# nagadomi/nunif

Measured on NVIDIA H100. Metric: waifu2x_input_megapixels_per_sec, higher is better.
Workload: dtype f16

## Files before the change

nunif_b200/csrc/gemm.cu:

```cuda
#include "gemm.h"
#include "gemm_wgmma.cuh"
#include "tmap.h"
#include "../../include/nunif_b200.h"
#include <mutex>
#include <cstdlib>

namespace nb200 {

typedef CUresult (*EncodeTiledFn)(CUtensorMap*, CUtensorMapDataType, cuuint32_t, void*, const cuuint64_t*,
                                  const cuuint64_t*, const cuuint32_t*, const cuuint32_t*, CUtensorMapInterleave,
                                  CUtensorMapSwizzle, CUtensorMapL2promotion, CUtensorMapFloatOOBfill);

static EncodeTiledFn get_encode() {
    static EncodeTiledFn fn = nullptr;
    static std::once_flag once;
    std::call_once(once, [] {
        void* p = nullptr;
        cudaDriverEntryPointQueryResult q;
        if (cudaGetDriverEntryPoint("cuTensorMapEncodeTiled", &p, cudaEnableDefault, &q) == cudaSuccess &&
            q == cudaDriverEntryPointSuccess)
            fn = (EncodeTiledFn)p;
    });
    return fn;
}

int encode(CUtensorMap* m, const void* base, int rank, const cuuint64_t* dims, const cuuint64_t* strides_bytes,
                  const cuuint32_t* box, int swizzle_bytes) {
    EncodeTiledFn fn = get_encode();
    if (!fn) return fail("cuTensorMapEncodeTiled is not available (no CUDA driver?)");
    cuuint32_t estr[5] = {1, 1, 1, 1, 1};
    CUtensorMapSwizzle sw = swizzle_bytes == 128 ? CU_TENSOR_MAP_SWIZZLE_128B
                                                 : (swizzle_bytes == 64 ? CU_TENSOR_MAP_SWIZZLE_64B : CU_TENSOR_MAP_SWIZZLE_32B);
    CUresult r = fn(m, CU_TENSOR_MAP_DATA_TYPE_FLOAT16, (cuuint32_t)rank, const_cast<void*>(base), dims, strides_bytes, box,
                    estr, CU_TENSOR_MAP_INTERLEAVE_NONE, sw, CU_TENSOR_MAP_L2_PROMOTION_L2_256B,
                    CU_TENSOR_MAP_FLOAT_OOB_FILL_NONE);
    if (r != CUDA_SUCCESS) return fail("cuTensorMapEncodeTiled failed with CUresult " + std::to_string((int)r));
    return 0;
}

template <int BN, int BK, bool A2 = false>
static int launch_t(cudaStream_t st, const GemmMaps& maps, const GemmParams& p, int m_tiles, int n_tiles) {
    using Cfg = GemmCfg<BN, BK>;
    if (ensure_dyn_smem((const void*)gemm_conv_kernel<BN, BK, A2>, Cfg::SMEM_BYTES)) return 1;
    cudaLaunchConfig_t cfg = {};
    cfg.gridDim = dim3((unsigned)m_tiles * n_tiles); cfg.blockDim = dim3(GEMM_THREADS); cfg.dynamicSmemBytes = Cfg::SMEM_BYTES;
    cfg.stream = st;
    cudaLaunchAttribute at[1];
    at[0].id = cudaLaunchAttributeProgrammaticStreamSerialization;
    at[0].val.programmaticStreamSerializationAllowed = 1;
    cfg.attrs = at; cfg.numAttrs = 1;
    NB_CUDA(cudaLaunchKernelEx(&cfg, gemm_conv_kernel<BN, BK, A2>, maps, p));
    NB_LAUNCHED();
    return 0;
}

template <int BK>
static int launch_bn(int bn, cudaStream_t st, const GemmMaps& maps, const GemmParams& p, int m_tiles, int n_tiles) {
    if (p.k2) switch (bn) {
        case 64: return launch_t<64, BK, true>(st, maps, p, m_tiles, n_tiles);
        case 96: return launch_t<96, BK, true>(st, maps, p, m_tiles, n_tiles);
        default: return fail("second A operand: unsupported BLOCK_N");
    }
    switch (bn) {
        case 16: return launch_t<16, BK>(st, maps, p, m_tiles, n_tiles);
        case 32: return launch_t<32, BK>(st, maps, p, m_tiles, n_tiles);
        case 48: return launch_t<48, BK>(st, maps, p, m_tiles, n_tiles);
        case 64: return launch_t<64, BK>(st, maps, p, m_tiles, n_tiles);
        case 96: return launch_t<96, BK>(st, maps, p, m_tiles, n_tiles);
        case 128: return launch_t<128, BK>(st, maps, p, m_tiles, n_tiles);
    }
    return fail("unsupported BLOCK_N");
}

static int num_sms() { return device_sm_count(); }

std::atomic<int> g_tune_epoch{0};
int g_tune[16] = {0, 0, 0,  0, 0, 0,  0,
                   0, 0,  0, 0, 0, 0, 0, 0, 0};

static int encode_nhwc4(CUtensorMap* m, const __half* base, int C, int X, int Y, int B, long long sx, long long sy, long long sb,
                        int cw, int tw, int th) {
    cuuint64_t dims[4] = {(cuuint64_t)C, (cuuint64_t)X, (cuuint64_t)Y, (cuuint64_t)B};
    cuuint64_t strides[3] = {(cuuint64_t)sx * 2, (cuuint64_t)sy * 2, (cuuint64_t)sb * 2};
    cuuint32_t box[4] = {(cuuint32_t)cw, (cuuint32_t)tw, (cuuint32_t)th, 1};
    return encode(m, base, 4, dims, strides, box, cw * 2);
}

int conv_gemm(cudaStream_t st, const ConvGemm& g) {
    NB_CHECK(g.A && g.Wt && g.out, "null pointer");
    NB_CHECK(g.Ci % 8 == 0, "input channel stride must be a multiple of 8");
    NB_CHECK(g.N % 16 == 0, "N must be a multiple of 16 (pad the weights)");
    GemmParams p;
    memset(&p, 0, sizeof(p));
    int ktap;
    cuuint64_t dims[5], strides[4];
    cuuint32_t box[5];
    const cuuint64_t e = 2;
    const cuuint64_t rs = (g.a_row_stride ? (cuuint64_t)g.a_row_stride : (cuuint64_t)g.Wi * g.Ci) * e;
    const cuuint64_t is = (g.a_img_stride ? (cuuint64_t)g.a_img_stride * e : (cuuint64_t)g.Hi * rs);
    switch (g.kind) {
        case CG_LINEAR_FLAT: {
            const long long M = (long long)g.B * g.Hi * g.Wi;
            p.B = 1; p.Ho = 1; p.Wo = (int)M; p.TH = 1; p.TW = 128;
            p.taps = g.a_planes; ktap = g.Cin;
            NB_CHECK(g.a_planes >= 1 && g.a_planes <= 16, "bad plane count");
            for (int t = 0; t < p.taps; ++t) { p.tap_dy[t] = 0; p.tap_dx[t] = 0; p.tap_dyi[t] = (int8_t)t; }
            dims[0] = g.Cin; dims[1] = M; dims[2] = g.a_planes; dims[3] = 1; dims[4] = 1;
            strides[0] = g.Ci * e; strides[1] = (g.a_planes > 1 ? (cuuint64_t)g.a_plane_stride : (cuuint64_t)M * g.Ci) * e;
            strides[2] = (cuuint64_t)M * g.Ci * e * g.a_planes; strides[3] = strides[2];
            break;
        }
        case CG_LINEAR_2D:
        case CG_CONV3: {
            const int kk = g.kind == CG_CONV3 ? 3 : 1;
            const int pad = g.kind == CG_CONV3 ? g.pad : 0;
            NB_CHECK(pad == 0 || pad == 1, "conv3x3 padding must be 0 or 1");
            p.B = g.B; p.Ho = g.Hi - (kk - 1) + 2 * pad; p.Wo = g.Wi - (kk - 1) + 2 * pad; p.TH = 8; p.TW = 16;
            p.taps = kk * kk; ktap = g.Cin;
            for (int t = 0; t < p.taps; ++t) { p.tap_dy[t] = (int8_t)(t / kk - pad); p.tap_dx[t] = (int8_t)(t % kk - pad); p.tap_dyi[t] = 0; }
            dims[0] = g.Cin; dims[1] = g.Wi; dims[2] = 1; dims[3] = g.Hi; dims[4] = g.B;
            strides[0] = g.Ci * e; strides[1] = rs; strides[2] = rs;
            strides[3] = is;
            break;
        }
        case CG_TCONV3: {
            NB_CHECK(g.dil >= 1 && g.dil <= 127, "temporal dilation must be in [1, 127]");
            p.B = g.B; p.Ho = g.Hi; p.Wo = g.Wi; p.TH = 8; p.TW = 16;
            p.taps = 3; ktap = g.Cin;
            for (int t = 0; t < 3; ++t) { p.tap_dy[t] = (int8_t)((t - 1) * g.dil); p.tap_dx[t] = 0; p.tap_dyi[t] = 0; }
            dims[0] = g.Cin; dims[1] = g.Wi; dims[2] = 1; dims[3] = g.Hi; dims[4] = g.B;
            strides[0] = g.Ci * e; strides[1] = rs; strides[2] = rs;
            strides[3] = is;
            break;
        }
        case CG_DOWN2: {
            NB_CHECK(g.Hi % 2 == 0 && g.Wi % 2 == 0, "2x2 stride-2 conv needs even H and W");
            NB_CHECK(g.Cin == g.Ci, "2x2 stride-2 conv needs a dense channel dimension");
            p.B = g.B; p.Ho = g.Hi / 2; p.Wo = g.Wi / 2; p.TH = 8; p.TW = 16;
            p.taps = 2; ktap = 2 * g.Cin;
            for (int t = 0; t < 2; ++t) { p.tap_dy[t] = 0; p.tap_dx[t] = 0; p.tap_dyi[t] = t; }
            dims[0] = 2 * g.Cin; dims[1] = g.Wi / 2; dims[2] = 2; dims[3] = g.Hi / 2; dims[4] = g.B;
            strides[0] = 2 * g.Ci * e; strides[1] = rs; strides[2] = 2 * rs;
            strides[3] = is;
            break;
        }
        default: return fail("conv_gemm: unknown kind");
    }
    NB_CHECK(ktap % 32 == 0, "K per tap must be a multiple of 32");
    const bool a2 = g.A2 != nullptr;
    if (a2) {
        NB_CHECK(g.out_mode == OUT_PIXSHUF2 && !g.res, "a second A operand needs the pixel-shuffle output and no residual");
        NB_CHECK(g.Cin2 > 0 && g.Cin2 % 32 == 0 && g.Cin2 <= g.ld2 && g.ld2 % 8 == 0, "second A operand: bad channel count");
    }
    const int BK = (ktap % 64 == 0 && g.Cin2 % 64 == 0) ? 64 : 32;
    p.cpt = ktap / BK;
    p.k2 = a2 ? g.Cin2 / BK : 0;
    p.tiles_x = cdiv(p.Wo, p.TW);
    p.tiles_y = cdiv(p.Ho, p.TH);
    p.N = g.N;
    p.bias = g.bias; p.act = g.act; p.out_mode = g.out_mode; p.cout = g.cout;
    p.has_res = g.res ? 1 : 0;
    p.res_before_act = g.res_before_act;
    const bool shuf = g.out_mode == OUT_PIXSHUF2;
    const bool split = g.out_mode == OUT_SPLIT;
    if (split) {
        NB_CHECK(g.cout % 16 == 0 && g.N % g.cout == 0 && g.N / g.cout <= 4, "split output: N must be 1..4 blocks of cout");
        NB_CHECK(!g.res, "split output does not take a residual");
    }
    if (shuf) {
        NB_CHECK(g.kind != CG_LINEAR_FLAT, "pixel-shuffle output needs 2-D tiling");
        NB_CHECK(g.cout % 16 == 0 && g.N == 4 * g.cout, "pixel-shuffle: N must be 4*cout, cout % 16 == 0");
    }
    NB_CHECK(g.ldo % 8 == 0 && (!g.res || g.ldr % 8 == 0), "channel strides must be multiples of 8");
    int bn = 0, cw = 0;
    static const int cands[] = {128, 96, 64, 48, 32, 16};
    for (int c : cands) {
        const int w = (c % 64 == 0) ? 64 : ((c % 32 == 0) ? 32 : 16);
        if (g.N % c == 0 && (!shuf || g.cout % w == 0) && (!split || g.cout % c == 0) && (!a2 || ((c == 96 || c == 64) && g.cout % c == 0))) {
            bn = c; cw = w; break;
        }
    }
    NB_CHECK(bn > 0, "no BLOCK_N divides N");
    if (!shuf) {
        const long long m_tiles_est = (long long)p.tiles_x * p.tiles_y * p.B;
        static const int narrower[] = {96, 64};
        for (int c : narrower) {
            if ((long long)(g.N / bn) * m_tiles_est >= (long long)num_sms() * 3 / 4) break;
            if (c >= bn || g.N % c) continue;
            const int w = (c % 64 == 0) ? 64 : 32;
            if (split && g.cout % w) continue;
            bn = c; cw = w;
        }
    }
    p.n_tiles = g.N / bn;
    box[0] = BK; box[1] = p.TW; box[2] = 1; box[3] = p.TH; box[4] = 1;
    GemmMaps maps;
    memset(&maps, 0, sizeof(maps));
    if (encode(&maps.a, g.A, 5, dims, strides, box, BK * 2)) return 1;
    const int K = p.taps * ktap + (a2 ? g.Cin2 : 0);
    cuuint64_t bdims[2] = {(cuuint64_t)K, (cuuint64_t)g.N};
    cuuint64_t bstr[1] = {(cuuint64_t)K * e};
    cuuint32_t bbox[2] = {(cuuint32_t)BK, (cuuint32_t)bn};
    if (encode(&maps.b, g.Wt, 2, bdims, bstr, bbox, BK * 2)) return 1;
    if (split) {
        for (int q = 0; q < g.N / g.cout; ++q)
            if (encode_nhwc4(&maps.o[q], g.out + (size_t)q * g.split_stride, g.cout, p.Wo, p.Ho, p.B, g.ldo, (long long)p.Wo * g.ldo,
                             (long long)p.Ho * p.Wo * g.ldo, cw, p.TW, p.TH)) return 1;
    } else if (!shuf) {
        if (encode_nhwc4(&maps.o[0], g.out, g.N, p.Wo, p.Ho, p.B, g.ldo, (long long)p.Wo * g.ldo, (long long)p.Ho * p.Wo * g.ldo,
                         cw, p.TW, p.TH)) return 1;
        if (g.res) {
            const int rW = g.kind == CG_LINEAR_FLAT ? p.Wo : g.res_W, rH = g.kind == CG_LINEAR_FLAT ? 1 : g.res_H;
            p.res_cx = g.kind == CG_LINEAR_FLAT ? 0 : g.res_cx;
            p.res_cy = g.kind == CG_LINEAR_FLAT ? 0 : g.res_cy;
            if (encode_nhwc4(&maps.r[0], g.res, g.N, rW, rH, p.B, g.ldr, (long long)rW * g.ldr, (long long)rH * rW * g.ldr, cw,
                             p.TW, p.TH)) return 1;
        }
    } else {
        const int OW = 2 * p.Wo, OH = 2 * p.Ho;
        for (int q = 0; q < 4; ++q) {
            const int dy = q >> 1, dx = q & 1;
            if (encode_nhwc4(&maps.o[q], g.out + ((size_t)dy * OW + dx) * g.ldo, g.cout, p.Wo, p.Ho, p.B, 2LL * g.ldo,
                             2LL * OW * g.ldo, (long long)OH * OW * g.ldo, cw, p.TW, p.TH)) return 1;
            if (g.res) {
                const int oy = dy + g.res_cy, ox = dx + g.res_cx;
                NB_CHECK(oy + 2 * (p.Ho - 1) < g.res_H && ox + 2 * (p.Wo - 1) < g.res_W, "residual tensor too small");
                if (encode_nhwc4(&maps.r[q], g.res + ((size_t)oy * g.res_W + ox) * g.ldr, g.cout, p.Wo, p.Ho, p.B, 2LL * g.ldr,
                                 2LL * g.res_W * g.ldr, (long long)g.res_H * g.res_W * g.ldr, cw, p.TW, p.TH)) return 1;
            }
        }
        p.res_cx = p.res_cy = 0;
        if (a2) {
            const cuuint64_t px = (cuuint64_t)g.ld2 * e;
            cuuint64_t d2[5] = {(cuuint64_t)g.Cin2, 2, (cuuint64_t)p.Wo, 2, (cuuint64_t)p.B * p.Ho};
            cuuint64_t s2[4] = {px, 2 * px, (cuuint64_t)OW * px, 2 * (cuuint64_t)OW * px};
            cuuint32_t b2[5] = {(cuuint32_t)BK, 1, (cuuint32_t)p.TW, 1, (cuuint32_t)p.TH};
            if (encode(&maps.a2, g.A2, 5, d2, s2, b2, BK * 2)) return 1;
        }
    }
    const int m_tiles = p.tiles_x * p.tiles_y * p.B;
    const double Mrows = (double)p.B * p.Ho * p.Wo;
    const double in_px = g.kind == CG_DOWN2 ? 4.0 * Mrows : ((g.kind == CG_CONV3 || g.kind == CG_TCONV3) ? (double)p.B * g.Hi * g.Wi : Mrows);
    ProfScope ps(st, PC_GEMM, 2.0 * Mrows * (double)g.N * (double)K,
                 in_px * (g.kind == CG_LINEAR_FLAT ? g.Cin * g.a_planes : g.Cin) * 2.0 + (g.res ? Mrows * g.N * 2.0 : 0.0) +
                     4.0 * Mrows * g.Cin2 * (a2 ? 2.0 : 0.0) + (double)g.N * K * 2.0,
                 Mrows * (double)g.N * 2.0);
    if (rec_on()) {
        char line[512];
        snprintf(line, sizeof(line),
                 "gemm,%d,%d,%d,%d,%d,%d,%d,%d,%lld,%lld,%d,%lld,%d,%d,%d,%d,%d,%lld,%d,%d,%d,%d,%d,%d,%d,%d,%d,%d,%d,%d,%d,%d,%d,%d",
                 g.kind, g.pad, g.dil, g.B, g.Hi, g.Wi, g.Ci, g.Cin, g.a_row_stride, g.a_img_stride, g.a_planes, g.a_plane_stride,
                 g.N, g.act, g.ldo, g.out_mode, g.cout, g.split_stride, g.bias ? 1 : 0, g.res ? 1 : 0, g.ldr, g.res_H, g.res_W,
                 g.res_cy, g.res_cx, g.res_before_act, a2 ? 1 : 0, g.Cin2, g.ld2, g.res && (const void*)g.out == (const void*)g.res,
                 (const void*)g.out == (const void*)g.A, bn, BK, m_tiles * p.n_tiles);
        rec_append(line);
    }
    return BK == 64 ? launch_bn<64>(bn, st, maps, p, m_tiles, p.n_tiles) : launch_bn<32>(bn, st, maps, p, m_tiles, p.n_tiles);
}

}

using namespace nb200;

extern "C" int nb200_conv_gemm_f16(const void* A, int B, int Hi, int Wi, int Ci, int Cin, int kind, const void* Wt, int N,
                                   const float* bias, int act, void* out, int ldo, int out_mode, int cout,
                                   const void* res, int ldr, int res_H, int res_W, int res_cy, int res_cx,
                                   int res_before_act, void* stream) {
    ConvGemm g;
    g.A = (const __half*)A; g.B = B; g.Hi = Hi; g.Wi = Wi; g.Ci = Ci; g.Cin = Cin;
    g.kind = kind == 4 ? CG_CONV3 : kind;
    g.pad = kind == 4 ? 1 : 0;
    g.Wt = (const __half*)Wt; g.N = N; g.bias = bias; g.act = act; g.out = (__half*)out; g.ldo = ldo;
    g.out_mode = out_mode; g.cout = cout; g.res = (const __half*)res; g.ldr = ldr; g.res_H = res_H; g.res_W = res_W;
    g.res_cy = res_cy; g.res_cx = res_cx; g.res_before_act = res_before_act;
    return conv_gemm((cudaStream_t)stream, g);
}

extern "C" int nb200_conv_gemm_pixshuf_a2_f16(const void* A, int B, int Hi, int Wi, int Ci, const void* Wt, int N, const float* bias,
                                              int act, void* out, int ldo, int cout, const void* A2, int Cin2, int ld2, void* stream) {
    ConvGemm g;
    g.A = (const __half*)A; g.B = B; g.Hi = Hi; g.Wi = Wi; g.Ci = Ci; g.Cin = Ci; g.kind = CG_LINEAR_2D;
    g.Wt = (const __half*)Wt; g.N = N; g.bias = bias; g.act = act; g.out = (__half*)out; g.ldo = ldo;
    g.out_mode = OUT_PIXSHUF2; g.cout = cout; g.A2 = (const __half*)A2; g.Cin2 = Cin2; g.ld2 = ld2;
    NB_CHECK(g.A2, "null pointer");
    return conv_gemm((cudaStream_t)stream, g);
}

extern "C" int nb200_conv_gemm_ex_f16(const nb200_gemm_desc* d, const void* A, const void* Wt, const float* bias, void* out,
                                      const void* res, const void* A2, void* stream) {
    NB_CHECK(d, "null descriptor");
    ConvGemm g;
    g.A = (const __half*)A; g.B = d->B; g.Hi = d->Hi; g.Wi = d->Wi; g.Ci = d->Ci; g.Cin = d->Cin;
    g.a_row_stride = d->a_row_stride; g.a_img_stride = d->a_img_stride; g.kind = d->kind; g.pad = d->pad; g.dil = d->dil;
    g.Wt = (const __half*)Wt; g.N = d->N; g.bias = bias; g.act = d->act; g.out = (__half*)out; g.ldo = d->ldo;
    g.out_mode = d->out_mode; g.cout = d->cout; g.split_stride = d->split_stride; g.a_planes = d->a_planes;
    g.a_plane_stride = d->a_plane_stride; g.res = (const __half*)res; g.ldr = d->ldr; g.res_H = d->res_H; g.res_W = d->res_W;
    g.res_cy = d->res_cy; g.res_cx = d->res_cx; g.res_before_act = d->res_before_act;
    g.A2 = (const __half*)A2; g.Cin2 = d->Cin2; g.ld2 = d->ld2;
    return conv_gemm((cudaStream_t)stream, g);
}

extern "C" int nb200_tune_set(int key, int value) {
    NB_CHECK(key >= 0 && key < 16, "bad key");
    g_tune[key] = value;
    g_tune_epoch.fetch_add(1);
    return 0;
}
```

nunif_b200/csrc/swin_block.cu:

```cuda
#include "gemm_wgmma.cuh"
#include "swin_kernels.h"
#include "tmap.h"

namespace nb200 {

constexpr int FM_ROWS = 128, FM_STAGES = 5, FM_THREADS = GEMM_CONSUMER_THREADS + 128;
constexpr int FM_PRODUCER_REGS = 40, FM_CONSUMER_REGS = 232;

template <int C>
struct FmCfg {
    static constexpr int KB = C / 32;
    static constexpr int TILE = FM_ROWS * C * 2;
    static constexpr int STAGE = 128 * C;
    static constexpr int SMEM = 2 * TILE + FM_STAGES * STAGE + (2 * FM_STAGES + KB + 1) * 8 + 1024;
};

struct FmMaps {
    CUtensorMap x, att, wp, w1, w2, y, wy;
};

template <int K>
__device__ __forceinline__ float (&half96(float (&acc)[K], int h))[48] { return *reinterpret_cast<float(*)[48]>(&acc[48 * h]); }

__device__ __forceinline__ void wgmma_wait_n(int n) {
    if (n == 0) wgmma_wait<0>();
    else wgmma_wait<1>();
}

template <int C, bool PROJ, int CS>
__global__ void __launch_bounds__(FM_THREADS, 1) swin_mlp_fused_kernel(const __grid_constant__ FmMaps maps, const float* __restrict__ bp,
                                                                     const float* __restrict__ b1, const float* __restrict__ b2,
                                                                     const float* __restrict__ by) {
    using Cfg = FmCfg<C>;
    static_assert(CS % 16 == 0 && 2 * C * CS <= Cfg::STAGE && CS * 256 <= Cfg::TILE, "Wy must fit a ring stage, y the att tile");
    constexpr int KB = Cfg::KB, NP = (KB + 1) / 2, NH = 2 * C / 64, NHALF = C / 96;
    extern __shared__ uint8_t smem_dyn[];
    uint8_t* smem = reinterpret_cast<uint8_t*>((reinterpret_cast<uintptr_t>(smem_dyn) + 1023) & ~(uintptr_t)1023);
    uint8_t* sx = smem;
    uint8_t* satt = smem + Cfg::TILE;
    uint8_t* ring = smem + 2 * Cfg::TILE;
    uint64_t* full = reinterpret_cast<uint64_t*>(ring + FM_STAGES * Cfg::STAGE);
    uint64_t* empty = full + FM_STAGES;
    uint64_t* abar = empty + FM_STAGES;
    uint64_t* xbar = abar + KB;
    const int tid = threadIdx.x, warp = tid >> 5;
    const int row_base = blockIdx.x * FM_ROWS;
    if (tid == GEMM_CONSUMER_THREADS) {
        tma_prefetch_desc(&maps.x);
        tma_prefetch_desc(&maps.w1);
        tma_prefetch_desc(&maps.w2);
        if (CS) tma_prefetch_desc(&maps.wy);
        if (PROJ) {
            tma_prefetch_desc(&maps.att);
            tma_prefetch_desc(&maps.wp);
        }
        for (int s = 0; s < FM_STAGES; ++s) {
            mbar_init(&full[s], 1);
            mbar_init(&empty[s], 2);
        }
        for (int kb = 0; kb < KB; ++kb) mbar_init(&abar[kb], 1);
        mbar_init(xbar, 1);
        fence_barrier_init();
    }
    __syncthreads();

    if (warp >= GEMM_CONSUMER_THREADS / 32) {
        asm volatile("setmaxnreg.dec.sync.aligned.u32 %0;" ::"n"(FM_PRODUCER_REGS));
        if (warp == GEMM_CONSUMER_THREADS / 32 && elect_one()) {
            bool acts = false;
            auto load_acts = [&]() {
                asm volatile("griddepcontrol.wait;" ::: "memory");
                if (PROJ)
                    for (int kb = 0; kb < KB; ++kb) {
                        mbar_expect_tx(&abar[kb], FM_ROWS * 64);
                        tma_load_2d(&maps.att, &abar[kb], satt + kb * (FM_ROWS * 64), kb * 32, row_base);
                    }
                mbar_expect_tx(xbar, Cfg::TILE);
                for (int kb = 0; kb < KB; ++kb) tma_load_2d(&maps.x, xbar, sx + kb * (FM_ROWS * 64), kb * 32, row_base);
                acts = true;
            };
            int it = 0;
            auto push = [&](const CUtensorMap* m, int k0, int n0, int rows, int nbox) {
                if (it == FM_STAGES) load_acts();
                const int s = it % FM_STAGES;
                mbar_wait(&empty[s], ((it / FM_STAGES) & 1) ^ 1);
                mbar_expect_tx(&full[s], nbox * rows * 64);
                for (int b = 0; b < nbox; ++b) tma_load_2d(m, &full[s], ring + s * Cfg::STAGE + b * rows * 64, k0 + 32 * b, n0);
                ++it;
            };
            if (PROJ)
                for (int j = 0; j < NP; ++j) push(&maps.wp, 64 * j, 0, C, min(2, KB - 2 * j));
            push(&maps.w1, 0, 0, 64, KB);
            for (int hc = 0; hc < NH; ++hc) {
                if (hc + 1 < NH) push(&maps.w1, 0, (hc + 1) * 64, 64, KB);
                push(&maps.w2, hc * 64, 0, C, 2);
            }
            if (CS) push(&maps.wy, 0, 0, CS, KB);
            if (!acts) load_acts();
        }
        return;
    }

    asm volatile("setmaxnreg.inc.sync.aligned.u32 %0;" ::"n"(FM_CONSUMER_REGS));
    const int wg = tid >> 7, t = tid & 127;
    const int row0 = wg * 64 + (t >> 5) * 16 + ((t & 31) >> 2);
    const int cq = 2 * (t & 3);
    const uint32_t x_base = smem_u32(sx) + wg * 64 * 64, att_base = smem_u32(satt) + wg * 64 * 64;
    int it = 0, pending = 0;
    auto take = [&]() -> uint32_t {
        const int s = it % FM_STAGES;
        mbar_wait(&full[s], (it / FM_STAGES) & 1);
        return smem_u32(ring + s * Cfg::STAGE);
    };
    auto commit = [&]() {
        wgmma_commit();
        ++it;
        ++pending;
    };
    auto retire = [&](int n) {
        wgmma_wait_n(n);
#pragma unroll
        for (int k = 0; k < FM_STAGES; ++k)
            if (k < pending - n && t == 0) mbar_arrive(&empty[(it - pending + k) % FM_STAGES]);
        pending = min(pending, n);
    };

    if (PROJ) {
        float acc[C / 2];
#pragma unroll
        for (int j = 0; j < C / 2; ++j) acc[j] = 0.f;
        wgmma_fence_operands(acc);
#pragma unroll
        for (int j = 0; j < NP; ++j) {
            const uint32_t bb = take();
#pragma unroll
            for (int kb = 2 * j; kb < 2 * j + 2 && kb < KB; ++kb) mbar_wait(&abar[kb], 0);
            wgmma_fence();
#pragma unroll
            for (int kb = 2 * j; kb < 2 * j + 2 && kb < KB; ++kb) {
                const uint32_t a = att_base + kb * (FM_ROWS * 64), b = bb + (kb - 2 * j) * (C * 64);
#pragma unroll
                for (int s = 0; s < 2; ++s)
#pragma unroll
                    for (int h = 0; h < NHALF; ++h)
                        wgmma_f16<96>(half96(acc, h), make_kmajor_desc<64>(a + 32 * s), make_kmajor_desc<64>(b + h * 96 * 64 + 32 * s), 1u);
            }
            commit();
            retire(1);
        }
        retire(0);
        wgmma_fence_operands(acc);
        mbar_wait(xbar, 0);
#pragma unroll
        for (int j = 0; j < C / 8; ++j) {
            const int col = 8 * j + cq;
            const float2 bq = __ldg(reinterpret_cast<const float2*>(bp + col));
#pragma unroll
            for (int i = 0; i < 2; ++i) {
                __half2* p = reinterpret_cast<__half2*>(sx + sw64_off<FM_ROWS>(row0 + 8 * i, col));
                const float2 xv = __half22float2(*p);
                *p = __floats2half2_rn(xv.x + (acc[4 * j + 2 * i] + bq.x), xv.y + (acc[4 * j + 2 * i + 1] + bq.y));
            }
        }
        fence_async_smem();
        asm volatile("bar.sync %0, 128;" ::"r"(2 + wg) : "memory");
    } else {
        mbar_wait(xbar, 0);
    }

    float oacc[C / 2];
#pragma unroll
    for (int j = 0; j < C / 2; ++j) oacc[j] = 0.f;
    wgmma_fence_operands(oacc);
    float hacc[2][32];
    uint32_t af[4][4];
    auto fc1 = [&](float (&h)[32]) {
#pragma unroll
        for (int j = 0; j < 32; ++j) h[j] = 0.f;
        wgmma_fence_operands(h);
        const uint32_t bb = take();
        wgmma_fence();
#pragma unroll
        for (int kb = 0; kb < KB; ++kb) {
            const uint32_t a = x_base + kb * (FM_ROWS * 64), b = bb + kb * (64 * 64);
            wgmma_f16<64>(h, make_kmajor_desc<64>(a), make_kmajor_desc<64>(b), 1u);
            wgmma_f16<64>(h, make_kmajor_desc<64>(a + 32), make_kmajor_desc<64>(b + 32), 1u);
        }
        commit();
    };
    fc1(hacc[0]);
#pragma unroll
    for (int hc = 0; hc < NH; ++hc) {
        const int buf = hc & 1;
        if (hc + 1 < NH) fc1(hacc[buf ^ 1]);
        retire(hc + 1 < NH ? 1 : 0);
        wgmma_fence_operands(hacc[buf]);
#pragma unroll
        for (int kk = 0; kk < 4; ++kk)
#pragma unroll
            for (int q = 0; q < 4; ++q) {
                const int j = 2 * kk + (q >> 1), i = q & 1;
                const float2 bq = __ldg(reinterpret_cast<const float2*>(b1 + 64 * hc + 8 * j + cq));
                af[kk][q] = pack_half2(gelu_erf(hacc[buf][4 * j + 2 * i] + bq.x), gelu_erf(hacc[buf][4 * j + 2 * i + 1] + bq.y));
            }
        const uint32_t bb = take();
        wgmma_fence();
#pragma unroll
        for (int kb = 0; kb < 2; ++kb)
#pragma unroll
            for (int s = 0; s < 2; ++s)
#pragma unroll
                for (int h = 0; h < NHALF; ++h)
                    wgmma_f16_rs96(half96(oacc, h), af[2 * kb + s], make_kmajor_desc<64>(bb + kb * (C * 64) + h * 96 * 64 + 32 * s), 1u);
        commit();
    }
    retire(0);
    wgmma_fence_operands(oacc);
#pragma unroll
    for (int j = 0; j < C / 8; ++j) {
        const int col = 8 * j + cq;
        const float2 bq = __ldg(reinterpret_cast<const float2*>(b2 + col));
#pragma unroll
        for (int i = 0; i < 2; ++i) {
            __half2* p = reinterpret_cast<__half2*>(sx + sw64_off<FM_ROWS>(row0 + 8 * i, col));
            const float2 xv = __half22float2(*p);
            *p = __floats2half2_rn(xv.x + (oacc[4 * j + 2 * i] + bq.x), xv.y + (oacc[4 * j + 2 * i + 1] + bq.y));
        }
    }
    fence_async_smem();
    if constexpr (CS > 0) {
        asm volatile("bar.sync %0, 128;" ::"r"(2 + wg) : "memory");
        float yacc[CS / 2];
#pragma unroll
        for (int j = 0; j < CS / 2; ++j) yacc[j] = 0.f;
        wgmma_fence_operands(yacc);
        const uint32_t bb = take();
        wgmma_fence();
#pragma unroll
        for (int kb = 0; kb < KB; ++kb) {
            const uint32_t a = x_base + kb * (FM_ROWS * 64), b = bb + kb * (CS * 64);
            wgmma_f16<CS>(yacc, make_kmajor_desc<64>(a), make_kmajor_desc<64>(b), 1u);
            wgmma_f16<CS>(yacc, make_kmajor_desc<64>(a + 32), make_kmajor_desc<64>(b + 32), 1u);
        }
        commit();
        retire(0);
        wgmma_fence_operands(yacc);
#pragma unroll
        for (int j = 0; j < CS / 8; ++j) {
            const int col = 8 * j + cq;
            const float2 bq = __ldg(reinterpret_cast<const float2*>(by + col));
#pragma unroll
            for (int i = 0; i < 2; ++i) {
                __half2* p = reinterpret_cast<__half2*>(satt + (col >> 4) * (FM_ROWS * 32) + stage_off<16>(row0 + 8 * i, (col & 15) >> 3) +
                                                        (col & 7) * 2);
                *p = __floats2half2_rn(yacc[4 * j + 2 * i] + bq.x, yacc[4 * j + 2 * i + 1] + bq.y);
            }
        }
        fence_async_smem();
    }
    consumer_bar_sync();
    if (tid == 0) {
        if constexpr (CS > 0)
            for (int c = 0; c < CS / 16; ++c) tma_store_2d(&maps.y, satt + c * (FM_ROWS * 32), 16 * c, row_base);
        else
            for (int kb = 0; kb < KB; ++kb) tma_store_2d(&maps.x, sx + kb * (FM_ROWS * 64), kb * 32, row_base);
        tma_store_commit();
        tma_store_wait_read();
    }
}

static int map2d(CUtensorMap* m, const void* base, int cols, long long rows, int box_rows) {
    const cuuint64_t dims[2] = {(cuuint64_t)cols, (cuuint64_t)rows};
    const cuuint64_t strides[1] = {(cuuint64_t)cols * 2};
    const cuuint32_t box[2] = {32, (cuuint32_t)box_rows};
    return encode(m, base, 2, dims, strides, box, 64);
}

template <int C, bool PROJ, int CS = 0>
static int launch_mlp(cudaStream_t st, unsigned grid, const FmMaps& maps, const float* bp, const float* b1, const float* b2,
                      const float* by = nullptr) {
    if (ensure_dyn_smem((const void*)swin_mlp_fused_kernel<C, PROJ, CS>, FmCfg<C>::SMEM)) return 1;
    cudaLaunchConfig_t cfg = {};
    cfg.gridDim = dim3(grid); cfg.blockDim = dim3(FM_THREADS); cfg.dynamicSmemBytes = FmCfg<C>::SMEM;
    cfg.stream = st;
    cudaLaunchAttribute at[1];
    at[0].id = cudaLaunchAttributeProgrammaticStreamSerialization;
    at[0].val.programmaticStreamSerializationAllowed = 1;
    cfg.attrs = at; cfg.numAttrs = 1;
    NB_CUDA(cudaLaunchKernelEx(&cfg, swin_mlp_fused_kernel<C, PROJ, CS>, maps, bp, b1, b2, by));
    NB_LAUNCHED();
    return 0;
}

int swin_mlp_fused(cudaStream_t st, __half* x, const __half* att, long long T, int C, const __half* wp, const float* bp,
                   const __half* w1, const float* b1, const __half* w2, const float* b2, __half* y, int cs, const __half* wy,
                   const float* by) {
    NB_CHECK(x && w1 && b1 && w2 && b2 && (!att || (wp && bp)) && (!y || (att && wy && by)), "null pointer");
    NB_CHECK(C == 96 || C == 192, "C must be 96 or 192");
    NB_CHECK(!y || (C == 192 && cs == 48) || (C == 96 && cs == 16), "y: cs must be 48 at C = 192 and 16 at C = 96");
    NB_CHECK(T > 0 && T < (1LL << 31), "token count out of range");
    FmMaps maps;
    memset(&maps, 0, sizeof(maps));
    if (map2d(&maps.x, x, C, T, FM_ROWS)) return 1;
    if (att && (map2d(&maps.att, att, C, T, FM_ROWS) || map2d(&maps.wp, wp, C, C, C))) return 1;
    if (map2d(&maps.w1, w1, C, 2 * C, 64) || map2d(&maps.w2, w2, 2 * C, C, C)) return 1;
    if (y) {
        if (map2d(&maps.wy, wy, C, cs, cs)) return 1;
        const cuuint64_t dims[2] = {(cuuint64_t)cs, (cuuint64_t)T};
        const cuuint64_t strides[1] = {(cuuint64_t)cs * 2};
        const cuuint32_t box[2] = {16, FM_ROWS};
        if (encode(&maps.y, y, 2, dims, strides, box, 32)) return 1;
    }
    const double Td = (double)T;
    ProfScope ps(st, PC_FUSED_MLP, Td * C * 2 * (C * ((att ? 1 : 0) + 4) + (y ? cs : 0)), Td * C * 2 * (att ? 2 : 1),
                 Td * (y ? cs : C) * 2);
    const unsigned grid = (unsigned)((T + FM_ROWS - 1) / FM_ROWS);
    if (rec_on()) {
        char line[96];
        snprintf(line, sizeof(line), "swin_mlp,%lld,%d,%d,%d", T, C, att ? 1 : 0, y ? cs : 0);
        rec_append(line);
    }
    if (y) return C == 96 ? launch_mlp<96, true, 16>(st, grid, maps, bp, b1, b2, by) : launch_mlp<192, true, 48>(st, grid, maps, bp, b1, b2, by);
    if (C == 96) return att ? launch_mlp<96, true>(st, grid, maps, bp, b1, b2) : launch_mlp<96, false>(st, grid, maps, bp, b1, b2);
    return att ? launch_mlp<192, true>(st, grid, maps, bp, b1, b2) : launch_mlp<192, false>(st, grid, maps, bp, b1, b2);
}

}

using namespace nb200;

extern "C" int nb200_swin_mlp_fused_f16(void* x, const void* att, long long T, int C, const void* wp, const float* bp,
                                        const void* w1, const float* b1, const void* w2, const float* b2, void* stream) {
    return swin_mlp_fused((cudaStream_t)stream, (__half*)x, (const __half*)att, T, C, (const __half*)wp, bp, (const __half*)w1, b1,
                          (const __half*)w2, b2, nullptr, 0, nullptr, nullptr);
}

extern "C" int nb200_swin_mlp_fused_y_f16(void* x, const void* att, long long T, int C, const void* wp, const float* bp,
                                          const void* w1, const float* b1, const void* w2, const float* b2, void* y, int cs,
                                          const void* wy, const float* by, void* stream) {
    NB_CHECK(y, "null pointer");
    return swin_mlp_fused((cudaStream_t)stream, (__half*)x, (const __half*)att, T, C, (const __half*)wp, bp, (const __half*)w1, b1,
                          (const __half*)w2, b2, (__half*)y, cs, (const __half*)wy, by);
}

extern "C" int nb200_swin_attn_fused_f16(const void* x, const void* wqkv, const float* bqkv, const float* bias_table, void* att,
                                         int B, int H, int W, int C, int shift, void* stream) {
    NB_CHECK(bias_table, "null pointer");
    cudaStream_t st = (cudaStream_t)stream;
    float* frag = nullptr;
    NB_CUDA(cudaMallocAsync((void**)&frag, BIAS_FRAG_FLOATS * sizeof(float), st));
    int rc = build_bias_frag(st, bias_table, frag);
    if (!rc) rc = swin_attn_fused(st, (const __half*)x, (const __half*)wqkv, bqkv, frag, (__half*)att, B, H, W, C, shift);
    cudaFreeAsync(frag, st);
    return rc;
}
```

Baseline: 78.59.

## Make fused Swin MLP kernel persistent with multi-buffered activation tiles

Turns the fused Swin MLP kernel into a persistent kernel. The grid is capped at the SM count (with an optional g_tune override), and each CTA loops over several 128-row tiles. A second producer warp now handles activation loads and output TMA stores, using 2–3 rotating tile buffers with new barriers, so loads of the next tile and stores of the previous tile overlap with compute. This removes per-CTA launch, prologue and weight-prefetch costs and the serialised load/compute/store of the old one-tile-per-CTA layout. In exchange it uses more shared memory and a more complex barrier protocol, which risks correctness or deadlock.

```diff
diff --git a/nunif_b200/csrc/gemm.cu b/nunif_b200/csrc/gemm.cu
--- a/nunif_b200/csrc/gemm.cu
+++ b/nunif_b200/csrc/gemm.cu
@@ -76,7 +76,8 @@
 
 std::atomic<int> g_tune_epoch{0};
 int g_tune[16] = {0, 0, 0,  0, 0, 0,  0,
-                   0, 0,  0, 0, 0, 0, 0, 0, 0};
+                   0, 0,  0,
+                   0, 0, 0, 0, 0, 0};
 
 static int encode_nhwc4(CUtensorMap* m, const __half* base, int C, int X, int Y, int B, long long sx, long long sy, long long sb,
                         int cw, int tw, int th) {
diff --git a/nunif_b200/csrc/swin_block.cu b/nunif_b200/csrc/swin_block.cu
--- a/nunif_b200/csrc/swin_block.cu
+++ b/nunif_b200/csrc/swin_block.cu
@@ -1,8 +1,11 @@
 #include "gemm_wgmma.cuh"
 #include "swin_kernels.h"
 #include "tmap.h"
+#include <algorithm>
 
 namespace nb200 {
+
+extern int g_tune[16];
 
 constexpr int FM_ROWS = 128, FM_STAGES = 5, FM_THREADS = GEMM_CONSUMER_THREADS + 128;
 constexpr int FM_PRODUCER_REGS = 40, FM_CONSUMER_REGS = 232;
@@ -10,9 +13,11 @@
 template <int C>
 struct FmCfg {
     static constexpr int KB = C / 32;
+    static constexpr int NBUF = C == 96 ? 3 : 2;
     static constexpr int TILE = FM_ROWS * C * 2;
     static constexpr int STAGE = 128 * C;
-    static constexpr int SMEM = 2 * TILE + FM_STAGES * STAGE + (2 * FM_STAGES + KB + 1) * 8 + 1024;
+    static constexpr int SMEM = NBUF * TILE + FM_STAGES * STAGE + (2 * FM_STAGES + NBUF * (KB + 2) + 1) * 8 + 1024;
+    static_assert(SMEM <= 232448, "shared memory per CTA exceeds the opt-in limit");
 };
 
 struct FmMaps {
@@ -30,26 +35,33 @@
 template <int C, bool PROJ, int CS>
 __global__ void __launch_bounds__(FM_THREADS, 1) swin_mlp_fused_kernel(const __grid_constant__ FmMaps maps, const float* __restrict__ bp,
                                                                      const float* __restrict__ b1, const float* __restrict__ b2,
-                                                                     const float* __restrict__ by) {
+                                                                     const float* __restrict__ by, int ntiles) {
     using Cfg = FmCfg<C>;
-    static_assert(CS % 16 == 0 && 2 * C * CS <= Cfg::STAGE && CS * 256 <= Cfg::TILE, "Wy must fit a ring stage, y the att tile");
-    constexpr int KB = Cfg::KB, NP = (KB + 1) / 2, NH = 2 * C / 64, NHALF = C / 96;
+    static_assert(CS % 16 == 0 && 2 * C * CS <= Cfg::STAGE && CS * 256 <= Cfg::TILE, "Wy must fit a ring stage, y a tile");
+    constexpr int KB = Cfg::KB, NP = (KB + 1) / 2, NH = 2 * C / 64, NHALF = C / 96, NBUF = Cfg::NBUF;
+    constexpr int SPT = (PROJ ? NP : 0) + 2 * NH + (CS ? 1 : 0);
+    static_assert(SPT > FM_STAGES, "the barrier protocol needs more stages per tile than the ring holds");
+    constexpr int XAHEAD = PROJ ? NBUF - 1 : NBUF;
     extern __shared__ uint8_t smem_dyn[];
-    uint8_t* smem = reinterpret_cast<uint8_t*>((reinterpret_cast<uintptr_t>(smem_dyn) + 1023) & ~(uintptr_t)1023);
-    uint8_t* sx = smem;
-    uint8_t* satt = smem + Cfg::TILE;
-    uint8_t* ring = smem + 2 * Cfg::TILE;
+    uint8_t* smem = smem_dyn + ((1024u - (smem_u32(smem_dyn) & 1023u)) & 1023u);
+    uint8_t* ring = smem + NBUF * Cfg::TILE;
     uint64_t* full = reinterpret_cast<uint64_t*>(ring + FM_STAGES * Cfg::STAGE);
     uint64_t* empty = full + FM_STAGES;
     uint64_t* abar = empty + FM_STAGES;
-    uint64_t* xbar = abar + KB;
+    uint64_t* xbar = abar + NBUF * KB;
+    uint64_t* outw = xbar + NBUF;
+    uint64_t* xfree = outw + NBUF;
+    auto buf = [&](int b) { return smem + b * Cfg::TILE; };
     const int tid = threadIdx.x, warp = tid >> 5;
-    const int row_base = blockIdx.x * FM_ROWS;
+    const int nt = (ntiles - (int)blockIdx.x + (int)gridDim.x - 1) / (int)gridDim.x;
     if (tid == GEMM_CONSUMER_THREADS) {
         tma_prefetch_desc(&maps.x);
         tma_prefetch_desc(&maps.w1);
         tma_prefetch_desc(&maps.w2);
-        if (CS) tma_prefetch_desc(&maps.wy);
+        if (CS) {
+            tma_prefetch_desc(&maps.wy);
+            tma_prefetch_desc(&maps.y);
+        }
         if (PROJ) {
             tma_prefetch_desc(&maps.att);
             tma_prefetch_desc(&maps.wp);
@@ -58,8 +70,12 @@
             mbar_init(&full[s], 1);
             mbar_init(&empty[s], 2);
         }
-        for (int kb = 0; kb < KB; ++kb) mbar_init(&abar[kb], 1);
-        mbar_init(xbar, 1);
+        for (int b = 0; b < NBUF; ++b) {
+            for (int kb = 0; kb < KB; ++kb) mbar_init(&abar[b * KB + kb], 1);
+            mbar_init(&xbar[b], 1);
+            mbar_init(&outw[b], 2);
+        }
+        mbar_init(xfree, 2);
         fence_barrier_init();
     }
     __syncthreads();
@@ -67,36 +83,56 @@
     if (warp >= GEMM_CONSUMER_THREADS / 32) {
         asm volatile("setmaxnreg.dec.sync.aligned.u32 %0;" ::"n"(FM_PRODUCER_REGS));
         if (warp == GEMM_CONSUMER_THREADS / 32 && elect_one()) {
-            bool acts = false;
-            auto load_acts = [&]() {
-                asm volatile("griddepcontrol.wait;" ::: "memory");
-                if (PROJ)
-                    for (int kb = 0; kb < KB; ++kb) {
-                        mbar_expect_tx(&abar[kb], FM_ROWS * 64);
-                        tma_load_2d(&maps.att, &abar[kb], satt + kb * (FM_ROWS * 64), kb * 32, row_base);
-                    }
-                mbar_expect_tx(xbar, Cfg::TILE);
-                for (int kb = 0; kb < KB; ++kb) tma_load_2d(&maps.x, xbar, sx + kb * (FM_ROWS * 64), kb * 32, row_base);
-                acts = true;
-            };
             int it = 0;
             auto push = [&](const CUtensorMap* m, int k0, int n0, int rows, int nbox) {
-                if (it == FM_STAGES) load_acts();
                 const int s = it % FM_STAGES;
                 mbar_wait(&empty[s], ((it / FM_STAGES) & 1) ^ 1);
                 mbar_expect_tx(&full[s], nbox * rows * 64);
                 for (int b = 0; b < nbox; ++b) tma_load_2d(m, &full[s], ring + s * Cfg::STAGE + b * rows * 64, k0 + 32 * b, n0);
                 ++it;
             };
-            if (PROJ)
-                for (int j = 0; j < NP; ++j) push(&maps.wp, 64 * j, 0, C, min(2, KB - 2 * j));
-            push(&maps.w1, 0, 0, 64, KB);
-            for (int hc = 0; hc < NH; ++hc) {
-                if (hc + 1 < NH) push(&maps.w1, 0, (hc + 1) * 64, 64, KB);
-                push(&maps.w2, hc * 64, 0, C, 2);
-            }
-            if (CS) push(&maps.wy, 0, 0, CS, KB);
-            if (!acts) load_acts();
+            for (int j = 0; j < nt; ++j) {
+                if (PROJ)
+                    for (int p = 0; p < NP; ++p) push(&maps.wp, 64 * p, 0, C, min(2, KB - 2 * p));
+                push(&maps.w1, 0, 0, 64, KB);
+                for (int hc = 0; hc < NH; ++hc) {
+                    if (hc + 1 < NH) push(&maps.w1, 0, (hc + 1) * 64, 64, KB);
+                    push(&maps.w2, hc * 64, 0, C, 2);
+                }
+                if (CS) push(&maps.wy, 0, 0, CS, KB);
+            }
+        } else if (warp == GEMM_CONSUMER_THREADS / 32 + 1 && elect_one()) {
+            auto row = [&](int j) { return ((int)blockIdx.x + j * (int)gridDim.x) * FM_ROWS; };
+            auto load_att = [&](int j) {
+                const int b = j % NBUF;
+                for (int kb = 0; kb < KB; ++kb) {
+                    mbar_expect_tx(&abar[b * KB + kb], FM_ROWS * 64);
+                    tma_load_2d(&maps.att, &abar[b * KB + kb], buf(b) + kb * (FM_ROWS * 64), kb * 32, row(j));
+                }
+            };
+            auto load_x = [&](int j) {
+                uint8_t* dst = buf((j + PROJ) % NBUF);
+                mbar_expect_tx(&xbar[j % NBUF], Cfg::TILE);
+                for (int kb = 0; kb < KB; ++kb) tma_load_2d(&maps.x, &xbar[j % NBUF], dst + kb * (FM_ROWS * 64), kb * 32, row(j));
+            };
+            asm volatile("griddepcontrol.wait;" ::: "memory");
+            if (PROJ) load_att(0);
+            for (int j = 0; j < XAHEAD && j < nt; ++j) load_x(j);
+            for (int j = 0; j < nt; ++j) {
+                if (PROJ) {
+                    mbar_wait(xfree, j & 1);
+                    if (j + 1 < nt) load_att(j + 1);
+                }
+                const int b = j % NBUF;
+                mbar_wait(&outw[b], (j / NBUF) & 1);
+                if constexpr (CS > 0)
+                    for (int c = 0; c < CS / 16; ++c) tma_store_2d(&maps.y, buf(b) + c * (FM_ROWS * 32), 16 * c, row(j));
+                else
+                    for (int kb = 0; kb < KB; ++kb) tma_store_2d(&maps.x, buf(b) + kb * (FM_ROWS * 64), kb * 32, row(j));
+                tma_store_commit();
+                tma_store_wait_read();
+                if (j + XAHEAD < nt) load_x(j + XAHEAD);
+            }
         }
         return;
     }
@@ -105,167 +141,172 @@
     const int wg = tid >> 7, t = tid & 127;
     const int row0 = wg * 64 + (t >> 5) * 16 + ((t & 31) >> 2);
     const int cq = 2 * (t & 3);
-    const uint32_t x_base = smem_u32(sx) + wg * 64 * 64, att_base = smem_u32(satt) + wg * 64 * 64;
-    int it = 0, pending = 0;
-    auto take = [&]() -> uint32_t {
-        const int s = it % FM_STAGES;
-        mbar_wait(&full[s], (it / FM_STAGES) & 1);
-        return smem_u32(ring + s * Cfg::STAGE);
-    };
-    auto commit = [&]() {
-        wgmma_commit();
-        ++it;
-        ++pending;
-    };
-    auto retire = [&](int n) {
-        wgmma_wait_n(n);
-#pragma unroll
-        for (int k = 0; k < FM_STAGES; ++k)
-            if (k < pending - n && t == 0) mbar_arrive(&empty[(it - pending + k) % FM_STAGES]);
-        pending = min(pending, n);
-    };
-
-    if (PROJ) {
-        float acc[C / 2];
-#pragma unroll
-        for (int j = 0; j < C / 2; ++j) acc[j] = 0.f;
-        wgmma_fence_operands(acc);
-#pragma unroll
-        for (int j = 0; j < NP; ++j) {
+#pragma unroll 1
+    for (int it0 = 0; (int)blockIdx.x + it0 / SPT * (int)gridDim.x < ntiles; it0 += SPT) {
+        const int j = it0 / SPT;
+        int it = it0;
+        const int b = j % NBUF;
+        const uint32_t par = (j / NBUF) & 1;
+        uint8_t* sx1 = buf(b);
+        const uint8_t* sxin = buf((j + PROJ) % NBUF);
+        const uint32_t x1_base = smem_u32(sx1) + wg * 64 * 64;
+        int pending = 0;
+        auto take = [&]() -> uint32_t {
+            const int s = it % FM_STAGES;
+            mbar_wait(&full[s], (it / FM_STAGES) & 1);
+            return smem_u32(ring + s * Cfg::STAGE);
+        };
+        auto commit = [&]() {
+            wgmma_commit();
+            ++it;
+            ++pending;
+        };
+        auto retire = [&](int n) {
+            wgmma_wait_n(n);
+#pragma unroll
+            for (int k = 0; k < FM_STAGES; ++k)
+                if (k < pending - n && t == 0) mbar_arrive(&empty[(it - pending + k) % FM_STAGES]);
+            pending = min(pending, n);
+        };
+
+        if (PROJ) {
+            float acc[C / 2];
+#pragma unroll
+            for (int i = 0; i < C / 2; ++i) acc[i] = 0.f;
+            wgmma_fence_operands(acc);
+#pragma unroll
+            for (int p = 0; p < NP; ++p) {
+                const uint32_t bb = take();
+#pragma unroll
+                for (int kb = 2 * p; kb < 2 * p + 2 && kb < KB; ++kb) mbar_wait(&abar[b * KB + kb], par);
+                wgmma_fence();
+#pragma unroll
+                for (int kb = 2 * p; kb < 2 * p + 2 && kb < KB; ++kb) {
+                    const uint32_t a = x1_base + kb * (FM_ROWS * 64), w = bb + (kb - 2 * p) * (C * 64);
+#pragma unroll
+                    for (int s = 0; s < 2; ++s)
+#pragma unroll
+                        for (int h = 0; h < NHALF; ++h)
+                            wgmma_f16<96>(half96(acc, h), make_kmajor_desc<64>(a + 32 * s), make_kmajor_desc<64>(w + h * 96 * 64 + 32 * s), 1u);
+                }
+                commit();
+                retire(1);
+            }
+            retire(0);
+            wgmma_fence_operands(acc);
+            mbar_wait(&xbar[b], par);
+#pragma unroll
+            for (int q = 0; q < C / 8; ++q) {
+                const int col = 8 * q + cq;
+                const float2 bq = __ldg(reinterpret_cast<const float2*>(bp + col));
+#pragma unroll
+                for (int i = 0; i < 2; ++i) {
+                    const uint32_t off = sw64_off<FM_ROWS>(row0 + 8 * i, col);
+                    const float2 xv = __half22float2(*reinterpret_cast<const __half2*>(sxin + off));
+                    *reinterpret_cast<__half2*>(sx1 + off) =
+                        __floats2half2_rn(xv.x + (acc[4 * q + 2 * i] + bq.x), xv.y + (acc[4 * q + 2 * i + 1] + bq.y));
+                }
+            }
+            fence_async_smem();
+            asm volatile("bar.sync %0, 128;" ::"r"(2 + wg) : "memory");
+            if (t == 0) mbar_arrive(xfree);
+        } else {
+            mbar_wait(&xbar[b], par);
+        }
+
+        float oacc[C / 2];
+#pragma unroll
+        for (int i = 0; i < C / 2; ++i) oacc[i] = 0.f;
+        wgmma_fence_operands(oacc);
+        float hacc[2][32];
+        uint32_t af[4][4];
+        auto fc1 = [&](float (&h)[32]) {
+#pragma unroll
+            for (int i = 0; i < 32; ++i) h[i] = 0.f;
+            wgmma_fence_operands(h);
             const uint32_t bb = take();
-#pragma unroll
-            for (int kb = 2 * j; kb < 2 * j + 2 && kb < KB; ++kb) mbar_wait(&abar[kb], 0);
             wgmma_fence();
 #pragma unroll
-            for (int kb = 2 * j; kb < 2 * j + 2 && kb < KB; ++kb) {
-                const uint32_t a = att_base + kb * (FM_ROWS * 64), b = bb + (kb - 2 * j) * (C * 64);
+            for (int kb = 0; kb < KB; ++kb) {
+                const uint32_t a = x1_base + kb * (FM_ROWS * 64), w = bb + kb * (64 * 64);
+                wgmma_f16<64>(h, make_kmajor_desc<64>(a), make_kmajor_desc<64>(w), 1u);
+                wgmma_f16<64>(h, make_kmajor_desc<64>(a + 32), make_kmajor_desc<64>(w + 32), 1u);
+            }
+            commit();
+        };
+        fc1(hacc[0]);
+#pragma unroll
+        for (int hc = 0; hc < NH; ++hc) {
+            const int hb = hc & 1;
+            if (hc + 1 < NH) fc1(hacc[hb ^ 1]);
+            retire(hc + 1 < NH ? 1 : 0);
+            wgmma_fence_operands(hacc[hb]);
+#pragma unroll
+            for (int kk = 0; kk < 4; ++kk)
+#pragma unroll
+                for (int q = 0; q < 4; ++q) {
+                    const int c8 = 2 * kk + (q >> 1), i = q & 1;
+                    const float2 bq = __ldg(reinterpret_cast<const float2*>(b1 + 64 * hc + 8 * c8 + cq));
+                    af[kk][q] = pack_half2(gelu_erf(hacc[hb][4 * c8 + 2 * i] + bq.x), gelu_erf(hacc[hb][4 * c8 + 2 * i + 1] + bq.y));
+                }
+            const uint32_t bb = take();
+            wgmma_fence();
+#pragma unroll
+            for (int kb = 0; kb < 2; ++kb)
 #pragma unroll
                 for (int s = 0; s < 2; ++s)
 #pragma unroll
                     for (int h = 0; h < NHALF; ++h)
-                        wgmma_f16<96>(half96(acc, h), make_kmajor_desc<64>(a + 32 * s), make_kmajor_desc<64>(b + h * 96 * 64 + 32 * s), 1u);
-            }
+                        wgmma_f16_rs96(half96(oacc, h), af[2 * kb + s], make_kmajor_desc<64>(bb + kb * (C * 64) + h * 96 * 64 + 32 * s), 1u);
             commit();
-            retire(1);
         }
         retire(0);
-        wgmma_fence_operands(acc);
-        mbar_wait(xbar, 0);
-#pragma unroll
-        for (int j = 0; j < C / 8; ++j) {
-            const int col = 8 * j + cq;
-            const float2 bq = __ldg(reinterpret_cast<const float2*>(bp + col));
+        wgmma_fence_operands(oacc);
+#pragma unroll
+        for (int q = 0; q < C / 8; ++q) {
+            const int col = 8 * q + cq;
+            const float2 bq = __ldg(reinterpret_cast<const float2*>(b2 + col));
 #pragma unroll
             for (int i = 0; i < 2; ++i) {
-                __half2* p = reinterpret_cast<__half2*>(sx + sw64_off<FM_ROWS>(row0 + 8 * i, col));
+                __half2* p = reinterpret_cast<__half2*>(sx1 + sw64_off<FM_ROWS>(row0 + 8 * i, col));
                 const float2 xv = __half22float2(*p);
-                *p = __floats2half2_rn(xv.x + (acc[4 * j + 2 * i] + bq.x), xv.y + (acc[4 * j + 2 * i + 1] + bq.y));
+                *p = __floats2half2_rn(xv.x + (oacc[4 * q + 2 * i] + bq.x), xv.y + (oacc[4 * q + 2 * i + 1] + bq.y));
             }
         }
         fence_async_smem();
+        if constexpr (CS > 0) {
+            asm volatile("bar.sync %0, 128;" ::"r"(2 + wg) : "memory");
+            float yacc[CS / 2];
+#pragma unroll
+            for (int i = 0; i < CS / 2; ++i) yacc[i] = 0.f;
+            wgmma_fence_operands(yacc);
+            const uint32_t bb = take();
+            wgmma_fence();
+#pragma unroll
+            for (int kb = 0; kb < KB; ++kb) {
+                const uint32_t a = x1_base + kb * (FM_ROWS * 64), w = bb + kb * (CS * 64);
+                wgmma_f16<CS>(yacc, make_kmajor_desc<64>(a), make_kmajor_desc<64>(w), 1u);
+                wgmma_f16<CS>(yacc, make_kmajor_desc<64>(a + 32), make_kmajor_desc<64>(w + 32), 1u);
+            }
+            commit();
+            retire(0);
+            wgmma_fence_operands(yacc);
+            consumer_bar_sync();
+#pragma unroll
+            for (int q = 0; q < CS / 8; ++q) {
+                const int col = 8 * q + cq;
+                const float2 bq = __ldg(reinterpret_cast<const float2*>(by + col));
+#pragma unroll
+                for (int i = 0; i < 2; ++i) {
+                    __half2* p = reinterpret_cast<__half2*>(sx1 + (col >> 4) * (FM_ROWS * 32) + stage_off<16>(row0 + 8 * i, (col & 15) >> 3) +
+                                                            (col & 7) * 2);
+                    *p = __floats2half2_rn(yacc[4 * q + 2 * i] + bq.x, yacc[4 * q + 2 * i + 1] + bq.y);
+                }
+            }
+            fence_async_smem();
+        }
         asm volatile("bar.sync %0, 128;" ::"r"(2 + wg) : "memory");
-    } else {
-        mbar_wait(xbar, 0);
-    }
-
-    float oacc[C / 2];
-#pragma unroll
-    for (int j = 0; j < C / 2; ++j) oacc[j] = 0.f;
-    wgmma_fence_operands(oacc);
-    float hacc[2][32];
-    uint32_t af[4][4];
-    auto fc1 = [&](float (&h)[32]) {
-#pragma unroll
-        for (int j = 0; j < 32; ++j) h[j] = 0.f;
-        wgmma_fence_operands(h);
-        const uint32_t bb = take();
-        wgmma_fence();
-#pragma unroll
-        for (int kb = 0; kb < KB; ++kb) {
-            const uint32_t a = x_base + kb * (FM_ROWS * 64), b = bb + kb * (64 * 64);
-            wgmma_f16<64>(h, make_kmajor_desc<64>(a), make_kmajor_desc<64>(b), 1u);
-            wgmma_f16<64>(h, make_kmajor_desc<64>(a + 32), make_kmajor_desc<64>(b + 32), 1u);
-        }
-        commit();
-    };
-    fc1(hacc[0]);
-#pragma unroll
-    for (int hc = 0; hc < NH; ++hc) {
-        const int buf = hc & 1;
-        if (hc + 1 < NH) fc1(hacc[buf ^ 1]);
-        retire(hc + 1 < NH ? 1 : 0);
-        wgmma_fence_operands(hacc[buf]);
-#pragma unroll
-        for (int kk = 0; kk < 4; ++kk)
-#pragma unroll
-            for (int q = 0; q < 4; ++q) {
-                const int j = 2 * kk + (q >> 1), i = q & 1;
-                const float2 bq = __ldg(reinterpret_cast<const float2*>(b1 + 64 * hc + 8 * j + cq));
-                af[kk][q] = pack_half2(gelu_erf(hacc[buf][4 * j + 2 * i] + bq.x), gelu_erf(hacc[buf][4 * j + 2 * i + 1] + bq.y));
-            }
-        const uint32_t bb = take();
-        wgmma_fence();
-#pragma unroll
-        for (int kb = 0; kb < 2; ++kb)
-#pragma unroll
-            for (int s = 0; s < 2; ++s)
-#pragma unroll
-                for (int h = 0; h < NHALF; ++h)
-                    wgmma_f16_rs96(half96(oacc, h), af[2 * kb + s], make_kmajor_desc<64>(bb + kb * (C * 64) + h * 96 * 64 + 32 * s), 1u);
-        commit();
-    }
-    retire(0);
-    wgmma_fence_operands(oacc);
-#pragma unroll
-    for (int j = 0; j < C / 8; ++j) {
-        const int col = 8 * j + cq;
-        const float2 bq = __ldg(reinterpret_cast<const float2*>(b2 + col));
-#pragma unroll
-        for (int i = 0; i < 2; ++i) {
-            __half2* p = reinterpret_cast<__half2*>(sx + sw64_off<FM_ROWS>(row0 + 8 * i, col));
-            const float2 xv = __half22float2(*p);
-            *p = __floats2half2_rn(xv.x + (oacc[4 * j + 2 * i] + bq.x), xv.y + (oacc[4 * j + 2 * i + 1] + bq.y));
-        }
-    }
-    fence_async_smem();
-    if constexpr (CS > 0) {
-        asm volatile("bar.sync %0, 128;" ::"r"(2 + wg) : "memory");
-        float yacc[CS / 2];
-#pragma unroll
-        for (int j = 0; j < CS / 2; ++j) yacc[j] = 0.f;
-        wgmma_fence_operands(yacc);
-        const uint32_t bb = take();
-        wgmma_fence();
-#pragma unroll
-        for (int kb = 0; kb < KB; ++kb) {
-            const uint32_t a = x_base + kb * (FM_ROWS * 64), b = bb + kb * (CS * 64);
-            wgmma_f16<CS>(yacc, make_kmajor_desc<64>(a), make_kmajor_desc<64>(b), 1u);
-            wgmma_f16<CS>(yacc, make_kmajor_desc<64>(a + 32), make_kmajor_desc<64>(b + 32), 1u);
-        }
-        commit();
-        retire(0);
-        wgmma_fence_operands(yacc);
-#pragma unroll
-        for (int j = 0; j < CS / 8; ++j) {
-            const int col = 8 * j + cq;
-            const float2 bq = __ldg(reinterpret_cast<const float2*>(by + col));
-#pragma unroll
-            for (int i = 0; i < 2; ++i) {
-                __half2* p = reinterpret_cast<__half2*>(satt + (col >> 4) * (FM_ROWS * 32) + stage_off<16>(row0 + 8 * i, (col & 15) >> 3) +
-                                                        (col & 7) * 2);
-                *p = __floats2half2_rn(yacc[4 * j + 2 * i] + bq.x, yacc[4 * j + 2 * i + 1] + bq.y);
-            }
-        }
-        fence_async_smem();
-    }
-    consumer_bar_sync();
-    if (tid == 0) {
-        if constexpr (CS > 0)
-            for (int c = 0; c < CS / 16; ++c) tma_store_2d(&maps.y, satt + c * (FM_ROWS * 32), 16 * c, row_base);
-        else
-            for (int kb = 0; kb < KB; ++kb) tma_store_2d(&maps.x, sx + kb * (FM_ROWS * 64), kb * 32, row_base);
-        tma_store_commit();
-        tma_store_wait_read();
+        if (t == 0) mbar_arrive(&outw[b]);
     }
 }
 
@@ -277,17 +318,19 @@
 }
 
 template <int C, bool PROJ, int CS = 0>
-static int launch_mlp(cudaStream_t st, unsigned grid, const FmMaps& maps, const float* bp, const float* b1, const float* b2,
+static int launch_mlp(cudaStream_t st, int ntiles, const FmMaps& maps, const float* bp, const float* b1, const float* b2,
                       const float* by = nullptr) {
     if (ensure_dyn_smem((const void*)swin_mlp_fused_kernel<C, PROJ, CS>, FmCfg<C>::SMEM)) return 1;
     cudaLaunchConfig_t cfg = {};
-    cfg.gridDim = dim3(grid); cfg.blockDim = dim3(FM_THREADS); cfg.dynamicSmemBytes = FmCfg<C>::SMEM;
+    int grid = std::min(ntiles, device_sm_count());
+    if (g_tune[10] > 0) grid = std::min(grid, g_tune[10]);
+    cfg.gridDim = dim3((unsigned)grid); cfg.blockDim = dim3(FM_THREADS); cfg.dynamicSmemBytes = FmCfg<C>::SMEM;
     cfg.stream = st;
     cudaLaunchAttribute at[1];
     at[0].id = cudaLaunchAttributeProgrammaticStreamSerialization;
     at[0].val.programmaticStreamSerializationAllowed = 1;
     cfg.attrs = at; cfg.numAttrs = 1;
-    NB_CUDA(cudaLaunchKernelEx(&cfg, swin_mlp_fused_kernel<C, PROJ, CS>, maps, bp, b1, b2, by));
+    NB_CUDA(cudaLaunchKernelEx(&cfg, swin_mlp_fused_kernel<C, PROJ, CS>, maps, bp, b1, b2, by, ntiles));
     NB_LAUNCHED();
     return 0;
 }
@@ -314,15 +357,15 @@
     const double Td = (double)T;
     ProfScope ps(st, PC_FUSED_MLP, Td * C * 2 * (C * ((att ? 1 : 0) + 4) + (y ? cs : 0)), Td * C * 2 * (att ? 2 : 1),
                  Td * (y ? cs : C) * 2);
-    const unsigned grid = (unsigned)((T + FM_ROWS - 1) / FM_ROWS);
+    const int ntiles = (int)((T + FM_ROWS - 1) / FM_ROWS);
     if (rec_on()) {
         char line[96];
         snprintf(line, sizeof(line), "swin_mlp,%lld,%d,%d,%d", T, C, att ? 1 : 0, y ? cs : 0);
         rec_append(line);
     }
-    if (y) return C == 96 ? launch_mlp<96, true, 16>(st, grid, maps, bp, b1, b2, by) : launch_mlp<192, true, 48>(st, grid, maps, bp, b1, b2, by);
-    if (C == 96) return att ? launch_mlp<96, true>(st, grid, maps, bp, b1, b2) : launch_mlp<96, false>(st, grid, maps, bp, b1, b2);
-    return att ? launch_mlp<192, true>(st, grid, maps, bp, b1, b2) : launch_mlp<192, false>(st, grid, maps, bp, b1, b2);
+    if (y) return C == 96 ? launch_mlp<96, true, 16>(st, ntiles, maps, bp, b1, b2, by) : launch_mlp<192, true, 48>(st, ntiles, maps, bp, b1, b2, by);
+    if (C == 96) return att ? launch_mlp<96, true>(st, ntiles, maps, bp, b1, b2) : launch_mlp<96, false>(st, ntiles, maps, bp, b1, b2);
+    return att ? launch_mlp<192, true>(st, ntiles, maps, bp, b1, b2) : launch_mlp<192, false>(st, ntiles, maps, bp, b1, b2);
 }
 
 }
```

New measurement: 81.93, median of 6. 4.3% higher.
